# DeepRec-AI/DeepRec

Measured on AMD Instinct MI355X. Metric: samples/sec (whole node) DLRM Criteo-TB-shaped synthetic, higher is better.
Workload: dtype bf16; 1 GPU; model=dlrm, global_batch=8192, seq_len=1, parallelism=single, hip_graph=True, optimizer=adamasync, embedding_dim=16, num_tables=26

## Files before the change

deeprec_amd/ops/hip/dense_kernels.hip:

```cpp

#include <torch/extension.h>
#include <ATen/hip/HIPContext.h>
#include <hip/hip_runtime.h>
#include <hip/hip_bf16.h>

#include <algorithm>
#include <cstdint>

namespace py = pybind11;

static inline hipStream_t dense_stream() {
  return at::hip::getCurrentHIPStreamMasqueradingAsCUDA().stream();
}

namespace {

using bf16 = __hip_bfloat16;
using bf16x8 = __attribute__((ext_vector_type(8))) short;
using f32x4 = __attribute__((ext_vector_type(4))) float;

__device__ __forceinline__ float bf2f_u16(short u) {
  union {
    unsigned int i;
    float f;
  } cv;
  cv.i = ((unsigned int)(unsigned short)u) << 16;
  return cv.f;
}

__device__ __forceinline__ short f2bf_u16(float f) {
  union {
    float f;
    unsigned int i;
  } cv;
  cv.f = f;
  unsigned int lsb = (cv.i >> 16) & 1;
  cv.i += 0x7fff + lsb;
  return (short)(cv.i >> 16);
}

__device__ __forceinline__ short act_grad_u16(short g, short o, int act) {
  const float ov = bf2f_u16(o);
  if (act == 1) return ov > 0.0f ? g : (short)0;
  return f2bf_u16(bf2f_u16(g) * ov * (1.0f - ov));
}

__device__ __forceinline__ bf16x8 load_frag_row(const short* __restrict__ src,
                                                int r, int k0, int rows,
                                                int cols) {
  bf16x8 out;
  if (r < rows && k0 + 7 < cols) {
    const short* p = src + (int64_t)r * cols + k0;
    out = *reinterpret_cast<const bf16x8*>(p);
  } else {
#pragma unroll
    for (int i = 0; i < 8; ++i) {
      short v = 0;
      if (r < rows && k0 + i < cols) v = src[(int64_t)r * cols + k0 + i];
      out[i] = v;
    }
  }
  return out;
}

__device__ __forceinline__ bf16x8 load_frag_col(const short* __restrict__ src,
                                                int c, int k0, int rows,
                                                int cols) {
  bf16x8 out;
#pragma unroll
  for (int i = 0; i < 8; ++i) {
    short v = 0;
    int r = k0 + i;
    if (r < rows && c < cols) v = src[(int64_t)r * cols + c];
    out[i] = v;
  }
  return out;
}

template <int MT>
__global__ void k_linear_fwd_t(const short* __restrict__ A,
                               const short* __restrict__ W,
                               const float* __restrict__ bias, int M, int N,
                               int K, int act, short* __restrict__ C) {
  const int lane = threadIdx.x & 63;
  const int wave = threadIdx.x >> 6;
  const int ntiles64 = (N + 63) / 64;
  const int m0 = (blockIdx.x / ntiles64) * 64 * MT + wave * 16 * MT;
  const int n0 = (blockIdx.x % ntiles64) * 64;
  if (m0 >= M) return;
  const int col_b = n0 + (lane & 15);
  const int kgrp = (lane >> 4) * 8;
  f32x4 acc[MT][4] = {};
  const int nt = min(4, (N - n0 + 15) / 16);
  for (int k0 = 0; k0 < K; k0 += 32) {
    bf16x8 a[MT];
#pragma unroll
    for (int r = 0; r < MT; ++r)
      a[r] = load_frag_row(A, m0 + r * 16 + (lane & 15), k0 + kgrp, M, K);
#pragma unroll
    for (int t = 0; t < 4; ++t) {
      if (t >= nt) break;
      bf16x8 b = load_frag_row(W, col_b + t * 16, k0 + kgrp, N, K);
#pragma unroll
      for (int r = 0; r < MT; ++r)
        acc[r][t] = __builtin_amdgcn_mfma_f32_16x16x32_bf16(a[r], b,
                                                            acc[r][t], 0, 0,
                                                            0);
    }
  }
  __shared__ short cstage[4][16][72];
  const bool full_tile =
      (MT == 1) && (n0 + 64 <= N) && (m0 + 16 <= M) && ((N & 7) == 0);
  if (full_tile) {
#pragma unroll
    for (int t = 0; t < 4; ++t) {
      const int cn = t * 16 + (lane & 15);
      const float bv = bias ? bias[n0 + cn] : 0.0f;
#pragma unroll
      for (int i = 0; i < 4; ++i) {
        float v = acc[0][t][i] + bv;
        if (act == 1 && v < 0.0f) v = 0.0f;
        else if (act == 2) v = 1.0f / (1.0f + __expf(-v));
        cstage[wave][(lane >> 4) * 4 + i][cn] = f2bf_u16(v);
      }
    }
    __builtin_amdgcn_s_waitcnt(0);
#pragma unroll
    for (int half = 0; half < 2; ++half) {
      const int row = half * 8 + (lane >> 3);
      const int c8 = (lane & 7) * 8;
      bf16x8 vreg;
#pragma unroll
      for (int j = 0; j < 8; ++j) vreg[j] = cstage[wave][row][c8 + j];
      *reinterpret_cast<bf16x8*>(
          C + (int64_t)(m0 + row) * N + n0 + c8) = vreg;
    }
    return;
  }
#pragma unroll
  for (int r = 0; r < MT; ++r) {
#pragma unroll
    for (int t = 0; t < 4; ++t) {
      if (t >= nt) break;
      const int cn = n0 + t * 16 + (lane & 15);
      if (cn >= N) continue;
      const float bv = bias ? bias[cn] : 0.0f;
#pragma unroll
      for (int i = 0; i < 4; ++i) {
        int cm = m0 + r * 16 + (lane >> 4) * 4 + i;
        if (cm >= M) continue;
        float v = acc[r][t][i] + bv;
        if (act == 1 && v < 0.0f) v = 0.0f;
        else if (act == 2) v = 1.0f / (1.0f + __expf(-v));
        C[(int64_t)cm * N + cn] = f2bf_u16(v);
      }
    }
  }
}

__global__ void k_linear_dx(const short* __restrict__ G,
                            const short* __restrict__ W, int M, int N, int K,
                            short* __restrict__ dX,
                            const short* __restrict__ prev_out,
                            int prev_act) {
  const int lane = threadIdx.x & 63;
  const int wave = threadIdx.x >> 6;
  const int ktiles64 = (K + 63) / 64;
  const int m0 = (blockIdx.x / ktiles64) * 64 + wave * 16;
  const int c0 = (blockIdx.x % ktiles64) * 64;
  if (m0 >= M) return;
  const int row_g = m0 + (lane & 15);
  const int col_w = c0 + (lane & 15);
  const int kgrp = (lane >> 4) * 8;
  f32x4 acc[4] = {{0.f, 0.f, 0.f, 0.f}, {0.f, 0.f, 0.f, 0.f},
                  {0.f, 0.f, 0.f, 0.f}, {0.f, 0.f, 0.f, 0.f}};
  const int kt = min(4, (K - c0 + 15) / 16);
  for (int n0 = 0; n0 < N; n0 += 32) {
    bf16x8 a = load_frag_row(G, row_g, n0 + kgrp, M, N);
#pragma unroll
    for (int t = 0; t < 4; ++t) {
      if (t >= kt) break;
      bf16x8 b = load_frag_col(W, col_w + t * 16, n0 + kgrp, N, K);
      acc[t] = __builtin_amdgcn_mfma_f32_16x16x32_bf16(a, b, acc[t], 0, 0,
                                                       0);
    }
  }
#pragma unroll
  for (int t = 0; t < 4; ++t) {
    if (t >= kt) break;
    const int ck = c0 + t * 16 + (lane & 15);
    if (ck >= K) continue;
#pragma unroll
    for (int i = 0; i < 4; ++i) {
      int cm = m0 + (lane >> 4) * 4 + i;
      if (cm >= M) continue;
      short v = f2bf_u16(acc[t][i]);
      if (prev_out)
        v = act_grad_u16(v, prev_out[(int64_t)cm * K + ck], prev_act);
      dX[(int64_t)cm * K + ck] = v;
    }
  }
}

constexpr int DX_NSUP = 256;
__global__ void k_linear_dx_lds(const short* __restrict__ G,
                                const short* __restrict__ W, int M, int N,
                                int K, short* __restrict__ dX,
                                const short* __restrict__ prev_out,
                                int prev_act) {
  __shared__ short wl[64][DX_NSUP + 8];
  const int lane = threadIdx.x & 63;
  const int wave = threadIdx.x >> 6;
  const int ktiles64 = (K + 63) / 64;
  const int m0 = (blockIdx.x / ktiles64) * 128 + wave * 32;
  const int c0 = (blockIdx.x % ktiles64) * 64;
  const int row_g0 = m0 + (lane & 15);
  const int row_g1 = m0 + 16 + (lane & 15);
  const int kgrp = (lane >> 4) * 8;
  const int kt = min(4, (K - c0 + 15) / 16);
  f32x4 acc[2][4] = {};
  for (int ns = 0; ns < N; ns += DX_NSUP) {
    const int nlen = min(DX_NSUP, N - ns);
    __syncthreads();
    {
      const int r = threadIdx.x >> 3;
      const int seg = threadIdx.x & 7;
      const int nstg = (nlen + 31) & ~31;
      for (int it = 0; it * 32 < nstg; ++it) {
        int n = it * 32 + r;
        bf16x8 v = load_frag_row(W, ns + n, c0 + seg * 8, N, K);
#pragma unroll
        for (int j = 0; j < 8; ++j) wl[seg * 8 + j][n] = v[j];
      }
    }
    __syncthreads();
    if (m0 >= M) continue;
    for (int n0 = 0; n0 < nlen; n0 += 32) {
      bf16x8 a0 = load_frag_row(G, row_g0, ns + n0 + kgrp, M, N);
      bf16x8 a1 = load_frag_row(G, row_g1, ns + n0 + kgrp, M, N);
#pragma unroll
      for (int t = 0; t < 4; ++t) {
        if (t >= kt) break;
        bf16x8 b = *reinterpret_cast<const bf16x8*>(
            &wl[t * 16 + (lane & 15)][n0 + kgrp]);
        acc[0][t] =
            __builtin_amdgcn_mfma_f32_16x16x32_bf16(a0, b, acc[0][t], 0, 0,
                                                    0);
        acc[1][t] =
            __builtin_amdgcn_mfma_f32_16x16x32_bf16(a1, b, acc[1][t], 0, 0,
                                                    0);
      }
    }
  }
  if (m0 >= M) return;
#pragma unroll
  for (int rg = 0; rg < 2; ++rg) {
#pragma unroll
    for (int t = 0; t < 4; ++t) {
      if (t >= kt) break;
      const int ck = c0 + t * 16 + (lane & 15);
      if (ck >= K) continue;
#pragma unroll
      for (int i = 0; i < 4; ++i) {
        int cm = m0 + rg * 16 + (lane >> 4) * 4 + i;
        if (cm >= M) continue;
        short v = f2bf_u16(acc[rg][t][i]);
        if (prev_out)
          v = act_grad_u16(v, prev_out[(int64_t)cm * K + ck], prev_act);
        dX[(int64_t)cm * K + ck] = v;
      }
    }
  }
}

__global__ void k_linear_dw_lds(const short* __restrict__ G,
                                const short* __restrict__ A, int M, int N,
                                int K, float* __restrict__ dW,
                                float* __restrict__ dbias) {
  constexpr int CH = 128;
  constexpr int KG = 64;
  constexpr int APAD = 8;
  __shared__ short a_l[CH][KG + APAD];
  __shared__ short g_l[CH][16 + APAD];
  __shared__ float bred[16];

  const int lane = threadIdx.x & 63;
  const int wave = threadIdx.x >> 6;
  const int tid = threadIdx.x;
  const int kgroups = (K + KG - 1) / KG;
  const int tiles_n = (N + 15) / 16;
  const int tile_id = blockIdx.x % (tiles_n * kgroups);
  const int chunk = blockIdx.x / (tiles_n * kgroups);
  const int n0 = (tile_id / kgroups) * 16;
  const int k0 = (tile_id % kgroups) * KG;
  const int mbeg = chunk * CH;

  {
    const int r_in_iter = tid >> 3;
    const int seg = tid & 7;
    for (int it = 0; it < CH / 32; ++it) {
      int r = it * 32 + r_in_iter;
      int m = mbeg + r;
      bf16x8 v = load_frag_row(A, m, k0 + seg * 8, M, K);
      *reinterpret_cast<bf16x8*>(&a_l[r][seg * 8]) = v;
    }
    const int r_g = tid >> 1;
    const int seg_g = tid & 1;
    bf16x8 v = load_frag_row(G, mbeg + r_g, n0 + seg_g * 8, M, N);
    *reinterpret_cast<bf16x8*>(&g_l[r_g][seg_g * 8]) = v;
  }
  __syncthreads();

  const int kw = wave * 16;
  const int col_a = kw + (lane & 15);
  const int col_g = lane & 15;
  const int kgrp = (lane >> 4) * 8;
  f32x4 acc = {0.f, 0.f, 0.f, 0.f};
  float bsum = 0.0f;
  const bool do_bias = (dbias != nullptr) && (k0 == 0) && (wave == 0);
#pragma unroll
  for (int ms = 0; ms < CH; ms += 32) {
    bf16x8 afrag, gfrag;
#pragma unroll
    for (int i = 0; i < 8; ++i) {
      int m = ms + kgrp + i;
      gfrag[i] = g_l[m][col_g];
      afrag[i] = a_l[m][col_a];
    }
    acc = __builtin_amdgcn_mfma_f32_16x16x32_bf16(gfrag, afrag, acc, 0, 0,
                                                  0);
    if (do_bias) {
#pragma unroll
      for (int i = 0; i < 8; ++i) bsum += bf2f_u16(gfrag[i]);
    }
  }
  const int ck = k0 + col_a;
  if (ck < K) {
#pragma unroll
    for (int i = 0; i < 4; ++i) {
      int cn = n0 + (lane >> 4) * 4 + i;
      if (cn >= N) continue;
      atomicAdd(&dW[(int64_t)cn * K + ck], acc[i]);
    }
  }
  if (do_bias) {
    float v = bsum;
    for (int off = 16; off < 64; off += 16)
      v += __shfl(bsum, (lane & 15) + off);
    if (lane < 16) {
      int cn = n0 + lane;
      if (cn < N) atomicAdd(&dbias[cn], v);
    }
  }
}

__global__ void k_linear_dw_lds64(const short* __restrict__ G,
                                  const short* __restrict__ A, int M, int N,
                                  int K, float* __restrict__ dW,
                                  float* __restrict__ dbias) {
  constexpr int CH = 128;
  __shared__ short a_l[CH][64 + 8];
  __shared__ short g_l[CH][64 + 8];
  const int lane = threadIdx.x & 63;
  const int wave = threadIdx.x >> 6;
  const int tid = threadIdx.x;
  const int kgroups = (K + 63) / 64;
  const int ngroups = (N + 63) / 64;
  const int tile_id = blockIdx.x % (ngroups * kgroups);
  const int chunk = blockIdx.x / (ngroups * kgroups);
  const int n0 = (tile_id / kgroups) * 64;
  const int k0 = (tile_id % kgroups) * 64;
  const int mbeg = chunk * CH;
  {
    const int r = tid >> 3, seg = tid & 7;
    for (int it = 0; it < CH / 32; ++it) {
      int rr = it * 32 + r;
      *reinterpret_cast<bf16x8*>(&a_l[rr][seg * 8]) =
          load_frag_row(A, mbeg + rr, k0 + seg * 8, M, K);
      *reinterpret_cast<bf16x8*>(&g_l[rr][seg * 8]) =
          load_frag_row(G, mbeg + rr, n0 + seg * 8, M, N);
    }
  }
  __syncthreads();
  const int col_g = wave * 16 + (lane & 15);
  const int kgrp = (lane >> 4) * 8;
  f32x4 acc[4] = {};
  float bsum = 0.0f;
  const bool do_bias = (dbias != nullptr) && (k0 == 0);
#pragma unroll
  for (int ms = 0; ms < CH; ms += 32) {
    bf16x8 gfrag;
#pragma unroll
    for (int i = 0; i < 8; ++i) gfrag[i] = g_l[ms + kgrp + i][col_g];
    if (do_bias) {
#pragma unroll
      for (int i = 0; i < 8; ++i) bsum += bf2f_u16(gfrag[i]);
    }
#pragma unroll
    for (int t = 0; t < 4; ++t) {
      bf16x8 afrag;
#pragma unroll
      for (int i = 0; i < 8; ++i)
        afrag[i] = a_l[ms + kgrp + i][t * 16 + (lane & 15)];
      acc[t] =
          __builtin_amdgcn_mfma_f32_16x16x32_bf16(gfrag, afrag, acc[t], 0,
                                                  0, 0);
    }
  }
#pragma unroll
  for (int t = 0; t < 4; ++t) {
    const int ck = k0 + t * 16 + (lane & 15);
    if (ck >= K) continue;
#pragma unroll
    for (int i = 0; i < 4; ++i) {
      int cn = n0 + wave * 16 + (lane >> 4) * 4 + i;
      if (cn >= N) continue;
      atomicAdd(&dW[(int64_t)cn * K + ck], acc[t][i]);
    }
  }
  if (do_bias) {
    float v = bsum;
    for (int off = 16; off < 64; off += 16)
      v += __shfl(bsum, (lane & 15) + off);
    const int cn = n0 + wave * 16 + (lane & 15);
    if (lane < 16 && cn < N) atomicAdd(&dbias[cn], v);
  }
}

__global__ void k_linear_dw_lds64t(const short* __restrict__ G,
                                   const short* __restrict__ A, int M, int N,
                                   int K, int cpb,
                                   float* __restrict__ dW,
                                   float* __restrict__ dbias) {
  constexpr int CH = 128;
  __shared__ short a_t[64][CH + 8];
  __shared__ short g_t[64][CH + 8];
  const int lane = threadIdx.x & 63;
  const int wave = threadIdx.x >> 6;
  const int tid = threadIdx.x;
  const int kgroups = (K + 63) / 64;
  const int ngroups = (N + 63) / 64;
  const int tile_id = blockIdx.x % (ngroups * kgroups);
  const int chunk0 = (blockIdx.x / (ngroups * kgroups)) * cpb;
  const int n0 = (tile_id / kgroups) * 64;
  const int k0 = (tile_id % kgroups) * 64;
  const int col_g = wave * 16 + (lane & 15);
  const int kgrp = (lane >> 4) * 8;
  f32x4 acc[4] = {};
  float bsum = 0.0f;
  const bool do_bias = (dbias != nullptr) && (k0 == 0);
  for (int c = 0; c < cpb; ++c) {
    const int mbeg = (chunk0 + c) * CH;
    if (mbeg >= M) break;
    if (c > 0) __syncthreads();
    {
      const int r = tid >> 3, seg = tid & 7;
      for (int it = 0; it < CH / 32; ++it) {
        int rr = it * 32 + r;
        bf16x8 va = load_frag_row(A, mbeg + rr, k0 + seg * 8, M, K);
        bf16x8 vg = load_frag_row(G, mbeg + rr, n0 + seg * 8, M, N);
#pragma unroll
        for (int j = 0; j < 8; ++j) {
          a_t[seg * 8 + j][rr] = va[j];
          g_t[seg * 8 + j][rr] = vg[j];
        }
      }
    }
    __syncthreads();
#pragma unroll
    for (int ms = 0; ms < CH; ms += 32) {
      bf16x8 gfrag =
          *reinterpret_cast<const bf16x8*>(&g_t[col_g][ms + kgrp]);
      if (do_bias) {
#pragma unroll
        for (int i = 0; i < 8; ++i) bsum += bf2f_u16(gfrag[i]);
      }
#pragma unroll
      for (int t = 0; t < 4; ++t) {
        bf16x8 afrag = *reinterpret_cast<const bf16x8*>(
            &a_t[t * 16 + (lane & 15)][ms + kgrp]);
        acc[t] =
            __builtin_amdgcn_mfma_f32_16x16x32_bf16(gfrag, afrag, acc[t],
                                                    0, 0, 0);
      }
    }
  }
#pragma unroll
  for (int t = 0; t < 4; ++t) {
    const int ck = k0 + t * 16 + (lane & 15);
    if (ck >= K) continue;
#pragma unroll
    for (int i = 0; i < 4; ++i) {
      int cn = n0 + wave * 16 + (lane >> 4) * 4 + i;
      if (cn >= N) continue;
      atomicAdd(&dW[(int64_t)cn * K + ck], acc[t][i]);
    }
  }
  if (do_bias) {
    float v = bsum;
    for (int off = 16; off < 64; off += 16)
      v += __shfl(bsum, (lane & 15) + off);
    const int cn = n0 + wave * 16 + (lane & 15);
    if (lane < 16 && cn < N) atomicAdd(&dbias[cn], v);
  }
}

__device__ __forceinline__ float wave_sum(float v) {
#pragma unroll
  for (int off = 32; off; off >>= 1) v += __shfl_down(v, off);
  return __shfl(v, 0);
}

__global__ void k_l2norm_fwd(const short* __restrict__ X, int M, int N,
                             float eps, short* __restrict__ Y,
                             float* __restrict__ inv_norms) {
  const int lane = threadIdx.x & 63;
  const int row = blockIdx.x * 4 + (threadIdx.x >> 6);
  if (row >= M) return;
  const short* x = X + (int64_t)row * N;
  float ss = 0.0f;
  for (int j = lane; j < N; j += 64) {
    float v = bf2f_u16(x[j]);
    ss += v * v;
  }
  float inv = rsqrtf(fmaxf(wave_sum(ss), eps));
  short* y = Y + (int64_t)row * N;
  for (int j = lane; j < N; j += 64)
    y[j] = f2bf_u16(bf2f_u16(x[j]) * inv);
  if (lane == 0) inv_norms[row] = inv;
}

__global__ void k_l2norm_bwd(const short* __restrict__ dY,
                             const short* __restrict__ Y,
                             const float* __restrict__ inv_norms, int M,
                             int N, short* __restrict__ dX) {
  const int lane = threadIdx.x & 63;
  const int row = blockIdx.x * 4 + (threadIdx.x >> 6);
  if (row >= M) return;
  const short* dy = dY + (int64_t)row * N;
  const short* y = Y + (int64_t)row * N;
  float dot = 0.0f;
  for (int j = lane; j < N; j += 64)
    dot += bf2f_u16(y[j]) * bf2f_u16(dy[j]);
  dot = wave_sum(dot);
  const float inv = inv_norms[row];
  short* dx = dX + (int64_t)row * N;
  for (int j = lane; j < N; j += 64)
    dx[j] = f2bf_u16((bf2f_u16(dy[j]) - bf2f_u16(y[j]) * dot) * inv);
}

__global__ void k_zero_f32d(float* __restrict__ p, int64_t n) {
  const int64_t to16 =
      (int64_t)((16 - (reinterpret_cast<uintptr_t>(p) & 15)) & 15) >> 2;
  const int64_t head = to16 < n ? to16 : n;
  const int64_t nbody = (n - head) & ~3LL;
  float* body = p + head;
  int64_t i = (blockIdx.x * (int64_t)blockDim.x + threadIdx.x) * 4;
  int64_t stride = gridDim.x * (int64_t)blockDim.x * 4;
  for (; i < nbody; i += stride)
    *reinterpret_cast<float4*>(body + i) = make_float4(0.f, 0.f, 0.f, 0.f);
  if (blockIdx.x == 0 && threadIdx.x == 0) {
    for (int64_t j = 0; j < head; ++j) p[j] = 0.0f;
    for (int64_t j = head + nbody; j < n; ++j) p[j] = 0.0f;
  }
}

__global__ void k_dense_adam(float* __restrict__ w,
                             const float* __restrict__ g,
                             float* __restrict__ m, float* __restrict__ v,
                             short* __restrict__ w16,
                             const float* __restrict__ powers, int64_t n,
                             float lr, float beta1, float beta2, float eps,
                             float gscale) {
  const float lr_t = lr * sqrtf(1.0f - powers[1]) / (1.0f - powers[0]);
  int64_t i = blockIdx.x * (int64_t)blockDim.x + threadIdx.x;
  int64_t stride = gridDim.x * (int64_t)blockDim.x;
  for (; i < n; i += stride) {
    float gi = g[i] * gscale;
    float mn = beta1 * m[i] + (1.0f - beta1) * gi;
    float vn = beta2 * v[i] + (1.0f - beta2) * gi * gi;
    m[i] = mn;
    v[i] = vn;
    float wn = w[i] - lr_t * mn / (sqrtf(vn) + eps);
    w[i] = wn;
    if (w16) w16[i] = f2bf_u16(wn);
  }
}

template <int N>
__global__ void k_resln_fwd(const short* __restrict__ x,
                            const short* __restrict__ a,
                            const float* __restrict__ gamma,
                            const float* __restrict__ beta, int64_t M,
                            float eps, short* __restrict__ y,
                            short* __restrict__ z,
                            float* __restrict__ stats) {
  float gm[N], bt[N];
#pragma unroll
  for (int j = 0; j < N; ++j) {
    gm[j] = gamma[j];
    bt[j] = beta[j];
  }
  int64_t r = blockIdx.x * (int64_t)blockDim.x + threadIdx.x;
  int64_t stride = gridDim.x * (int64_t)blockDim.x;
  for (; r < M; r += stride) {
    const short* xp = x + r * N;
    const short* ap = a + r * N;
    float zv[N];
    float mean = 0.0f;
#pragma unroll
    for (int j = 0; j < N; ++j) {
      zv[j] = bf2f_u16(xp[j]) + bf2f_u16(ap[j]);
      mean += zv[j];
    }
    mean /= N;
    float var = 0.0f;
#pragma unroll
    for (int j = 0; j < N; ++j) {
      float d = zv[j] - mean;
      var += d * d;
    }
    float rstd = rsqrtf(var / N + eps);
    short* yp = y + r * N;
    short* zp = z + r * N;
#pragma unroll
    for (int j = 0; j < N; ++j) {
      zp[j] = f2bf_u16(zv[j]);
      yp[j] = f2bf_u16((zv[j] - mean) * rstd * gm[j] + bt[j]);
    }
    stats[r * 2] = mean;
    stats[r * 2 + 1] = rstd;
  }
}

template <int N>
__global__ void k_resln_bwd(const short* __restrict__ dy,
                            const short* __restrict__ z,
                            const float* __restrict__ stats,
                            const float* __restrict__ gamma, int64_t M,
                            short* __restrict__ dz,
                            float* __restrict__ dgamma,
                            float* __restrict__ dbeta) {
  __shared__ float ldg[N];
  __shared__ float ldb[N];
  for (int j = threadIdx.x; j < N; j += blockDim.x) {
    ldg[j] = 0.0f;
    ldb[j] = 0.0f;
  }
  __syncthreads();
  float gm[N], pg[N], pb[N];
#pragma unroll
  for (int j = 0; j < N; ++j) {
    gm[j] = gamma[j];
    pg[j] = 0.0f;
    pb[j] = 0.0f;
  }
  int64_t r = blockIdx.x * (int64_t)blockDim.x + threadIdx.x;
  int64_t stride = gridDim.x * (int64_t)blockDim.x;
  for (; r < M; r += stride) {
    const short* dyp = dy + r * N;
    const short* zp = z + r * N;
    const float mean = stats[r * 2];
    const float rstd = stats[r * 2 + 1];
    float s1 = 0.0f, s2 = 0.0f;
    float xh[N], g[N];
#pragma unroll
    for (int j = 0; j < N; ++j) {
      xh[j] = (bf2f_u16(zp[j]) - mean) * rstd;
      g[j] = bf2f_u16(dyp[j]);
      float gg = g[j] * gm[j];
      s1 += gg;
      s2 += gg * xh[j];
      pg[j] += g[j] * xh[j];
      pb[j] += g[j];
    }
    s1 /= N;
    s2 /= N;
    short* dzp = dz + r * N;
#pragma unroll
    for (int j = 0; j < N; ++j)
      dzp[j] = f2bf_u16((g[j] * gm[j] - s1 - xh[j] * s2) * rstd);
  }
#pragma unroll
  for (int j = 0; j < N; ++j) {
    atomicAdd(&ldg[j], pg[j]);
    atomicAdd(&ldb[j], pb[j]);
  }
  __syncthreads();
  for (int j = threadIdx.x; j < N; j += blockDim.x) {
    atomicAdd(&dgamma[j], ldg[j]);
    atomicAdd(&dbeta[j], ldb[j]);
  }
}

__global__ void k_act_bwd(const short* __restrict__ dY,
                          const short* __restrict__ out, int64_t n, int act,
                          short* __restrict__ G) {
  int64_t i = (blockIdx.x * (int64_t)blockDim.x + threadIdx.x) * 8;
  int64_t stride = gridDim.x * (int64_t)blockDim.x * 8;
  for (; i + 7 < n; i += stride) {
    bf16x8 g = *reinterpret_cast<const bf16x8*>(dY + i);
    bf16x8 o = *reinterpret_cast<const bf16x8*>(out + i);
    bf16x8 r;
#pragma unroll
    for (int j = 0; j < 8; ++j) r[j] = act_grad_u16(g[j], o[j], act);
    *reinterpret_cast<bf16x8*>(G + i) = r;
  }
  if (blockIdx.x == 0 && threadIdx.x == 0) {
    for (int64_t j = n & ~7LL; j < n; ++j)
      G[j] = act_grad_u16(dY[j], out[j], act);
  }
}

__global__ void k_pad_cast_bf16(const float* __restrict__ x, int64_t M, int K,
                                int KP, short* __restrict__ y) {
  const int gpr = (KP + 7) / 8;
  const int64_t ngroups = M * gpr;
  int64_t gi = blockIdx.x * (int64_t)blockDim.x + threadIdx.x;
  const int64_t stride = gridDim.x * (int64_t)blockDim.x;
  for (; gi < ngroups; gi += stride) {
    const int64_t r = gi / gpr;
    const int c0 = (int)(gi % gpr) * 8;
    bf16x8 v;
#pragma unroll
    for (int j = 0; j < 8; ++j) {
      short b = 0;
      if (c0 + j < K) {
        const float f = x[r * K + c0 + j];
        b = f != f ? (short)0x7fc0 : f2bf_u16(f);
      }
      v[j] = b;
    }
    short* dst = y + r * KP + c0;
    if ((KP & 7) == 0) {
      *reinterpret_cast<bf16x8*>(dst) = v;
    } else {
#pragma unroll
      for (int j = 0; j < 8; ++j)
        if (c0 + j < KP) dst[j] = v[j];
    }
  }
}

__global__ void k_interact_fwd(const short* __restrict__ feats, int B, int F,
                               int D, int P, int P_pad,
                               short* __restrict__ out) {
  const int lane = threadIdx.x & 63;
  const int wave = threadIdx.x >> 6;
  const int b = blockIdx.x * 4 + wave;
  extern __shared__ short lds[];
  short* f = lds + wave * F * D;
  const bool active = b < B;
  if (active) {
    const short* src = feats + (int64_t)b * F * D;
    for (int t = lane; t * 8 < F * D; t += 64) {
      *reinterpret_cast<bf16x8*>(f + t * 8) =
          *reinterpret_cast<const bf16x8*>(src + t * 8);
    }
  }
  __syncthreads();
  if (!active) return;
  short* dst = reinterpret_cast<short*>(out) + (int64_t)b * P_pad;
  for (int p = lane; p < P_pad; p += 64) {
    if (p >= P) {
      dst[p] = 0;
      continue;
    }
    int i = 0, rem = p, row = F - 1;
    while (rem >= row) {
      rem -= row;
      --row;
      ++i;
    }
    int j = i + 1 + rem;
    float acc = 0.0f;
    const short* fi = f + i * D;
    const short* fj = f + j * D;
    for (int d = 0; d < D; ++d)
      acc += bf2f_u16(fi[d]) * bf2f_u16(fj[d]);
    dst[p] = f2bf_u16(acc);
  }
}

__global__ void k_interact_cat_fwd(const short* __restrict__ bot,
                                   const short* __restrict__ emb, int B,
                                   int Fe, int D, int P, int P_pad,
                                   short* __restrict__ out) {
  const int lane = threadIdx.x & 63;
  const int wave = threadIdx.x >> 6;
  const int b = blockIdx.x * 4 + wave;
  const int F = Fe + 1;
  extern __shared__ short lds[];
  short* f = lds + wave * F * D;
  const bool active = b < B;
  if (active) {
    const short* bsrc = bot + (int64_t)b * D;
    for (int t = lane; t * 8 < D; t += 64)
      *reinterpret_cast<bf16x8*>(f + t * 8) =
          *reinterpret_cast<const bf16x8*>(bsrc + t * 8);
    const short* esrc = emb + (int64_t)b * Fe * D;
    for (int t = lane; t * 8 < Fe * D; t += 64)
      *reinterpret_cast<bf16x8*>(f + D + t * 8) =
          *reinterpret_cast<const bf16x8*>(esrc + t * 8);
  }
  __syncthreads();
  if (!active) return;
  short* dst = reinterpret_cast<short*>(out) + (int64_t)b * (D + P_pad);
  for (int d = lane; d < D; d += 64) dst[d] = f[d];
  dst += D;
  for (int p = lane; p < P_pad; p += 64) {
    if (p >= P) {
      dst[p] = 0;
      continue;
    }
    int i = 0, rem = p, row = F - 1;
    while (rem >= row) {
      rem -= row;
      --row;
      ++i;
    }
    int j = i + 1 + rem;
    float acc = 0.0f;
    const short* fi = f + i * D;
    const short* fj = f + j * D;
    for (int d = 0; d < D; ++d)
      acc += bf2f_u16(fi[d]) * bf2f_u16(fj[d]);
    dst[p] = f2bf_u16(acc);
  }
}

__global__ void k_interact_cat_bwd(const short* __restrict__ grad,
                                   const short* __restrict__ bot,
                                   const short* __restrict__ emb, int B,
                                   int Fe, int D, int P, int P_pad,
                                   short* __restrict__ dbot,
                                   short* __restrict__ demb) {
  const int lane = threadIdx.x & 63;
  const int wave = threadIdx.x >> 6;
  const int b = blockIdx.x * 4 + wave;
  const int F = Fe + 1;
  extern __shared__ short lds[];
  short* f = lds + wave * (F * D + ((P + 7) & ~7));
  short* g = f + F * D;
  const bool active = b < B;
  if (active) {
    const short* bsrc = bot + (int64_t)b * D;
    for (int t = lane; t * 8 < D; t += 64)
      *reinterpret_cast<bf16x8*>(f + t * 8) =
          *reinterpret_cast<const bf16x8*>(bsrc + t * 8);
    const short* esrc = emb + (int64_t)b * Fe * D;
    for (int t = lane; t * 8 < Fe * D; t += 64)
      *reinterpret_cast<bf16x8*>(f + D + t * 8) =
          *reinterpret_cast<const bf16x8*>(esrc + t * 8);
    const short* gsrc = grad + (int64_t)b * (D + P_pad) + D;
    for (int t = lane; t < P; t += 64) g[t] = gsrc[t];
  }
  __shared__ short plut[40 * 40];
  for (int t = threadIdx.x; t < F * F; t += blockDim.x) {
    int i = t / F, j = t % F;
    int lo = i < j ? i : j, hi = i < j ? j : i;
    plut[t] = (short)(i == j ? -1
                             : lo * F - (lo * (lo + 1)) / 2 + (hi - lo - 1));
  }
  __syncthreads();
  if (!active) return;
  const short* gdirect = grad + (int64_t)b * (D + P_pad);
  short* db = dbot + (int64_t)b * D;
  short* de = demb + (int64_t)b * Fe * D;
  for (int t = lane; t < F * D; t += 64) {
    int i = t / D, d = t % D;
    float acc = 0.0f;
    const short* prow = &plut[i * F];
    const short* fd = f + d;
#pragma unroll 4
    for (int j = 0; j < F; ++j) {
      int p = prow[j];
      if (p < 0) continue;
      acc += bf2f_u16(g[p]) * bf2f_u16(fd[j * D]);
    }
    if (i == 0) {
      db[d] = f2bf_u16(acc + bf2f_u16(gdirect[d]));
    } else {
      de[(i - 1) * D + d] = f2bf_u16(acc);
    }
  }
}

__global__ void k_interact_bwd(const short* __restrict__ grad,
                               const short* __restrict__ feats, int B, int F,
                               int D, int P, int P_pad,
                               short* __restrict__ dfeats) {
  const int lane = threadIdx.x & 63;
  const int wave = threadIdx.x >> 6;
  const int b = blockIdx.x * 4 + wave;
  extern __shared__ short lds[];
  short* f = lds + wave * (F * D + ((P + 7) & ~7));
  short* g = f + F * D;
  const bool active = b < B;
  if (active) {
    const short* fsrc = feats + (int64_t)b * F * D;
    const short* gsrc = grad + (int64_t)b * P_pad;
    for (int t = lane; t * 8 < F * D; t += 64)
      *reinterpret_cast<bf16x8*>(f + t * 8) =
          *reinterpret_cast<const bf16x8*>(fsrc + t * 8);
    for (int t = lane; t < P; t += 64) g[t] = gsrc[t];
  }
  __shared__ short plut[40 * 40];
  for (int t = threadIdx.x; t < F * F; t += blockDim.x) {
    int i = t / F, j = t % F;
    int lo = i < j ? i : j, hi = i < j ? j : i;
    plut[t] = (short)(i == j ? -1
                             : lo * F - (lo * (lo + 1)) / 2 + (hi - lo - 1));
  }
  __syncthreads();
  if (!active) return;
  short* dst = reinterpret_cast<short*>(dfeats) + (int64_t)b * F * D;
  for (int t = lane; t < F * D; t += 64) {
    int i = t / D, d = t % D;
    float acc = 0.0f;
    const short* prow = &plut[i * F];
    const short* fd = f + d;
#pragma unroll 4
    for (int j = 0; j < F; ++j) {
      int p = prow[j];
      if (p < 0) continue;
      acc += bf2f_u16(g[p]) * bf2f_u16(fd[j * D]);
    }
    dst[t] = f2bf_u16(acc);
  }
}

}


static const short* bf_ptr(const torch::Tensor& t) {
  return reinterpret_cast<const short*>(t.data_ptr<at::BFloat16>());
}
static short* bf_ptr_mut(torch::Tensor& t) {
  return reinterpret_cast<short*>(t.data_ptr<at::BFloat16>());
}

static void check_bf16_matrix(const torch::Tensor& t, const char* op,
                              const char* name) {
  TORCH_CHECK(t.is_cuda(), op, ": ", name, " must be on the GPU");
  TORCH_CHECK(t.dim() == 2, op, ": ", name, " must be 2-D, got ", t.dim(),
              "-D");
  TORCH_CHECK(t.scalar_type() == torch::kBFloat16, op, ": ", name,
              " must be bfloat16, got ", t.scalar_type());
  TORCH_CHECK(t.is_contiguous(), op, ": ", name,
              " must be contiguous (row-major)");
}

torch::Tensor linear_fwd(torch::Tensor x, torch::Tensor w_bf16,
                         torch::Tensor bias, int64_t act,
                         int64_t variant) {
  check_bf16_matrix(x, "linear_fwd", "x");
  check_bf16_matrix(w_bf16, "linear_fwd", "w");
  TORCH_CHECK(x.size(1) == w_bf16.size(1), "linear_fwd: x is [M,",
              x.size(1), "] but w is [N,", w_bf16.size(1), "]");
  int M = x.size(0), K = x.size(1), N = w_bf16.size(0);
  TORCH_CHECK(!bias.defined() || bias.numel() == 0 ||
                  (bias.numel() == N && bias.is_contiguous()),
              "linear_fwd: bias must be empty or contiguous [N]");
  auto out = torch::empty({M, N}, x.options());
  int tiles_n = (N + 63) / 64;
  const float* bp =
      bias.defined() && bias.numel() ? bias.data_ptr<float>() : nullptr;
  if (variant < 0) variant = 0;
  if (variant == 1) {
    int blocks = ((M + 127) / 128) * tiles_n;
    k_linear_fwd_t<2><<<blocks, 256, 0, dense_stream()>>>(
        bf_ptr(x), bf_ptr(w_bf16), bp, M, N, K, (int)act, bf_ptr_mut(out));
  } else {
    int blocks = ((M + 63) / 64) * tiles_n;
    k_linear_fwd_t<1><<<blocks, 256, 0, dense_stream()>>>(
        bf_ptr(x), bf_ptr(w_bf16), bp, M, N, K, (int)act, bf_ptr_mut(out));
  }
  return out;
}

torch::Tensor linear_dx(torch::Tensor g, torch::Tensor w_bf16,
                        c10::optional<torch::Tensor> prev_out,
                        int64_t prev_act) {
  check_bf16_matrix(g, "linear_dx", "g");
  check_bf16_matrix(w_bf16, "linear_dx", "w");
  TORCH_CHECK(g.size(1) == w_bf16.size(0), "linear_dx: g is [M,", g.size(1),
              "] but w is [", w_bf16.size(0), ",K]");
  int M = g.size(0), N = g.size(1), K = w_bf16.size(1);
  TORCH_CHECK(prev_act >= 0 && prev_act <= 2, "linear_dx: prev_act must be "
              "0 (none), 1 (relu) or 2 (sigmoid), got ", prev_act);
  const short* pp = nullptr;
  if (prev_out.has_value()) {
    check_bf16_matrix(*prev_out, "linear_dx", "prev_out");
    TORCH_CHECK(prev_out->size(0) == M && prev_out->size(1) == K,
                "linear_dx: prev_out is [", prev_out->size(0), ",",
                prev_out->size(1), "] but dX is [", M, ",", K, "]");
    if (prev_act != 0) pp = bf_ptr(*prev_out);
  } else {
    TORCH_CHECK(prev_act == 0, "linear_dx: prev_act without prev_out");
  }
  auto dx = torch::empty({M, K}, g.options());
  int tiles_k = (K + 63) / 64;
  if (N >= 128) {
    int blocks = ((M + 127) / 128) * tiles_k;
    k_linear_dx_lds<<<blocks, 256, 0, dense_stream()>>>(
        bf_ptr(g), bf_ptr(w_bf16), M, N, K, bf_ptr_mut(dx), pp,
        (int)prev_act);
  } else {
    int blocks = ((M + 63) / 64) * tiles_k;
    k_linear_dx<<<blocks, 256, 0, dense_stream()>>>(
        bf_ptr(g), bf_ptr(w_bf16), M, N, K, bf_ptr_mut(dx), pp,
        (int)prev_act);
  }
  return dx;
}

static void zero_f32_launch(float* p, int64_t n) {
  k_zero_f32d<<<(int)std::clamp<int64_t>((n / 4 + 255) / 256, 1, 1024), 256,
                0, dense_stream()>>>(p, n);
}

static std::tuple<torch::Tensor, torch::Tensor> linear_dw_impl(
    torch::Tensor g, torch::Tensor x, torch::Tensor ws, bool want_bias,
    int64_t variant, bool zero = true) {
  check_bf16_matrix(g, "linear_dw", "g");
  check_bf16_matrix(x, "linear_dw", "x");
  TORCH_CHECK(g.size(0) == x.size(0), "linear_dw: g has ", g.size(0),
              " rows but x has ", x.size(0));
  int M = g.size(0), N = g.size(1), K = x.size(1);
  int64_t ws_len = (int64_t)N * K + (want_bias ? N : 0);
  if (zero) zero_f32_launch(ws.data_ptr<float>(), ws_len);
  auto dw = ws.narrow(0, 0, (int64_t)N * K).view({N, K});
  auto db = want_bias ? ws.narrow(0, (int64_t)N * K, N) : torch::Tensor();
  int m_chunks = (M + 127) / 128;
  float* dbp = want_bias ? db.data_ptr<float>() : nullptr;
  if (variant < 0) variant = N >= 64 ? 2 : 0;
  if (variant == 2) {
    int tiles = ((N + 63) / 64) * ((K + 63) / 64);
    int cpb = std::max(1, (int)((int64_t)m_chunks * tiles / 512));
    int chunk_blocks = (m_chunks + cpb - 1) / cpb;
    k_linear_dw_lds64t<<<tiles * chunk_blocks, 256, 0, dense_stream()>>>(
        bf_ptr(g), bf_ptr(x), M, N, K, cpb, dw.data_ptr<float>(), dbp);
  } else if (variant == 1) {
    int tiles = ((N + 63) / 64) * ((K + 63) / 64);
    k_linear_dw_lds64<<<tiles * m_chunks, 256, 0, dense_stream()>>>(
        bf_ptr(g), bf_ptr(x), M, N, K, dw.data_ptr<float>(), dbp);
  } else {
    int tiles = ((N + 15) / 16) * ((K + 63) / 64);
    k_linear_dw_lds<<<tiles * m_chunks, 256, 0, dense_stream()>>>(
        bf_ptr(g), bf_ptr(x), M, N, K, dw.data_ptr<float>(), dbp);
  }
  return {dw, db};
}

std::tuple<torch::Tensor, torch::Tensor> linear_dw(torch::Tensor g,
                                                   torch::Tensor x,
                                                   bool want_bias,
                                                   int64_t variant) {
  check_bf16_matrix(g, "linear_dw", "g");
  check_bf16_matrix(x, "linear_dw", "x");
  int N = g.size(1), K = x.size(1);
  int64_t ws_len = (int64_t)N * K + (want_bias ? N : 0);
  auto ws = torch::empty({ws_len}, g.options().dtype(torch::kFloat32));
  return linear_dw_impl(g, x, ws, want_bias, variant);
}

std::tuple<torch::Tensor, torch::Tensor> linear_dw_out(torch::Tensor g,
                                                       torch::Tensor x,
                                                       torch::Tensor ws,
                                                       bool want_bias,
                                                       int64_t variant,
                                                       bool zero) {
  TORCH_CHECK(ws.is_cuda() && ws.is_contiguous() &&
              ws.scalar_type() == torch::kFloat32);
  check_bf16_matrix(g, "linear_dw_out", "g");
  check_bf16_matrix(x, "linear_dw_out", "x");
  int N = g.size(1), K = x.size(1);
  int64_t ws_len = (int64_t)N * K + (want_bias ? N : 0);
  TORCH_CHECK(ws.numel() == ws_len, "linear_dw_out: workspace size");
  return linear_dw_impl(g, x, ws, want_bias, variant, zero);
}

void zero_f32(torch::Tensor ws) {
  TORCH_CHECK(ws.is_cuda() && ws.dim() == 1 && ws.is_contiguous() &&
                  ws.scalar_type() == torch::kFloat32,
              "zero_f32: ws must be a contiguous 1-D fp32 GPU tensor");
  if (ws.numel() == 0) return;
  zero_f32_launch(ws.data_ptr<float>(), ws.numel());
}

torch::Tensor pad_cast_bf16(torch::Tensor x, int64_t k_pad) {
  TORCH_CHECK(x.is_cuda() && x.dim() == 2 && x.is_contiguous() &&
                  x.scalar_type() == torch::kFloat32,
              "pad_cast_bf16: x must be a contiguous 2-D fp32 GPU tensor");
  int64_t M = x.size(0), K = x.size(1);
  TORCH_CHECK(k_pad >= K, "pad_cast_bf16: k_pad ", k_pad, " < K ", K);
  TORCH_CHECK(k_pad < (1 << 30), "pad_cast_bf16: k_pad ", k_pad,
              " is out of range (< 2^30)");
  auto y = torch::empty({M, k_pad}, x.options().dtype(torch::kBFloat16));
  if (M == 0 || k_pad == 0) return y;
  int64_t groups = M * ((k_pad + 7) / 8);
  int blocks = (int)std::clamp<int64_t>((groups + 255) / 256, 1, 4096);
  k_pad_cast_bf16<<<blocks, 256, 0, dense_stream()>>>(
      x.data_ptr<float>(), M, (int)K, (int)k_pad, bf_ptr_mut(y));
  return y;
}

std::tuple<torch::Tensor, torch::Tensor, torch::Tensor> resln_fwd(
    torch::Tensor x, torch::Tensor a, torch::Tensor gamma,
    torch::Tensor beta, double eps) {
  TORCH_CHECK(x.scalar_type() == torch::kBFloat16 && x.is_contiguous());
  int64_t M = x.numel() / x.size(-1);
  int N = x.size(-1);
  TORCH_CHECK(N <= 64, "resln: row width must be <= 64");
  auto y = torch::empty_like(x);
  auto z = torch::empty_like(x);
  auto stats = torch::empty({M, 2}, x.options().dtype(torch::kFloat32));
  if (M == 0) return {y, z, stats};
  TORCH_CHECK(N == 16 || N == 32 || N == 64, "resln: N must be 16/32/64");
  int blocks = (int)std::min<int64_t>((M + 255) / 256, 4096);
#define RESLN_FWD(NV) \
  k_resln_fwd<NV><<<blocks, 256, 0, dense_stream()>>>( \
      bf_ptr(x), bf_ptr(a), gamma.data_ptr<float>(), \
      beta.data_ptr<float>(), M, (float)eps, bf_ptr_mut(y), \
      bf_ptr_mut(z), stats.data_ptr<float>())
  if (N == 16) RESLN_FWD(16);
  else if (N == 32) RESLN_FWD(32);
  else RESLN_FWD(64);
#undef RESLN_FWD
  return {y, z, stats};
}

std::tuple<torch::Tensor, torch::Tensor, torch::Tensor> resln_bwd(
    torch::Tensor dy, torch::Tensor z, torch::Tensor stats,
    torch::Tensor gamma) {
  int64_t M = z.numel() / z.size(-1);
  int N = z.size(-1);
  auto dz = torch::empty_like(z);
  auto opts = gamma.options();
  auto dgamma = torch::empty({N}, opts);
  auto dbeta = torch::empty({N}, opts);
  auto stream = dense_stream();
  k_zero_f32d<<<1, 64, 0, stream>>>(dgamma.data_ptr<float>(), N);
  k_zero_f32d<<<1, 64, 0, stream>>>(dbeta.data_ptr<float>(), N);
  if (M == 0) return {dz, dgamma, dbeta};
  auto dyc = dy.contiguous();
  int blocks = (int)std::min<int64_t>((M + 256 * 8 - 1) / (256 * 8), 4096);
  blocks = std::max(blocks, 64);
#define RESLN_BWD(NV) \
  k_resln_bwd<NV><<<blocks, 256, 0, stream>>>( \
      bf_ptr(dyc), bf_ptr(z), stats.data_ptr<float>(), \
      gamma.data_ptr<float>(), M, bf_ptr_mut(dz), \
      dgamma.data_ptr<float>(), dbeta.data_ptr<float>())
  if (N == 16) RESLN_BWD(16);
  else if (N == 32) RESLN_BWD(32);
  else RESLN_BWD(64);
#undef RESLN_BWD
  return {dz, dgamma, dbeta};
}

void dense_adam(torch::Tensor w, torch::Tensor g, torch::Tensor m,
                torch::Tensor v, torch::Tensor w16, torch::Tensor powers,
                double lr, double beta1, double beta2, double eps,
                double gscale) {
  int64_t n = w.numel();
  if (n == 0) return;
  short* w16p = (w16.defined() && w16.numel())
                    ? reinterpret_cast<short*>(w16.data_ptr<at::BFloat16>())
                    : nullptr;
  int blocks = (int)std::min<int64_t>((n + 255) / 256, 4096);
  k_dense_adam<<<blocks, 256, 0, dense_stream()>>>(
      w.data_ptr<float>(), g.data_ptr<float>(), m.data_ptr<float>(),
      v.data_ptr<float>(), w16p, powers.data_ptr<float>(), n, (float)lr,
      (float)beta1, (float)beta2, (float)eps, (float)gscale);
}

torch::Tensor act_bwd(torch::Tensor dy, torch::Tensor out, int64_t act) {
  auto g = torch::empty_like(dy);
  int64_t n = dy.numel();
  int blocks = (int)std::min<int64_t>((n / 8 + 255) / 256, 4096);
  k_act_bwd<<<std::max(blocks, 1), 256, 0, dense_stream()>>>(
      bf_ptr(dy), bf_ptr(out), n, (int)act, bf_ptr_mut(g));
  return g;
}

torch::Tensor interact_fwd(torch::Tensor feats, int64_t p_pad) {
  TORCH_CHECK(feats.scalar_type() == torch::kBFloat16 &&
              feats.is_contiguous());
  int B = feats.size(0), F = feats.size(1), D = feats.size(2);
  int P = F * (F - 1) / 2;
  TORCH_CHECK((F * D) % 8 == 0, "F*D must be a multiple of 8");
  auto out = torch::empty({B, p_pad}, feats.options());
  int blocks = (B + 3) / 4;
  size_t lds = 4 * (size_t)F * D * sizeof(short);
  k_interact_fwd<<<blocks, 256, lds, dense_stream()>>>(
      bf_ptr(feats), B, F, D, P, (int)p_pad, bf_ptr_mut(out));
  return out;
}

torch::Tensor interact_bwd(torch::Tensor grad, torch::Tensor feats) {
  int B = feats.size(0), F = feats.size(1), D = feats.size(2);
  TORCH_CHECK(F <= 40, "interact_bwd: pair LUT supports F <= 40");
  int P = F * (F - 1) / 2;
  int P_pad = grad.size(1);
  auto dfeats = torch::empty_like(feats);
  int blocks = (B + 3) / 4;
  size_t lds = 4 * (size_t)(F * D + ((P + 7) & ~7)) * sizeof(short);
  k_interact_bwd<<<blocks, 256, lds, dense_stream()>>>(
      bf_ptr(grad.contiguous()), bf_ptr(feats), B, F, D, P, P_pad,
      bf_ptr_mut(dfeats));
  return dfeats;
}

torch::Tensor interact_cat_fwd(torch::Tensor bot, torch::Tensor emb,
                               int64_t p_pad) {
  TORCH_CHECK(bot.scalar_type() == torch::kBFloat16 && bot.is_contiguous());
  TORCH_CHECK(emb.scalar_type() == torch::kBFloat16 && emb.is_contiguous());
  int B = emb.size(0), Fe = emb.size(1), D = emb.size(2);
  int F = Fe + 1;
  int P = F * (F - 1) / 2;
  TORCH_CHECK(D % 8 == 0, "D must be a multiple of 8");
  auto out = torch::empty({B, D + p_pad}, emb.options());
  int blocks = (B + 3) / 4;
  size_t lds = 4 * (size_t)F * D * sizeof(short);
  k_interact_cat_fwd<<<blocks, 256, lds, dense_stream()>>>(
      bf_ptr(bot), bf_ptr(emb), B, Fe, D, P, (int)p_pad, bf_ptr_mut(out));
  return out;
}

std::tuple<torch::Tensor, torch::Tensor> interact_cat_bwd(
    torch::Tensor grad, torch::Tensor bot, torch::Tensor emb) {
  int B = emb.size(0), Fe = emb.size(1), D = emb.size(2);
  int F = Fe + 1;
  TORCH_CHECK(F <= 40, "interact: pair LUT supports F <= 40");
  int P = F * (F - 1) / 2;
  int P_pad = grad.size(1) - D;
  auto dbot = torch::empty_like(bot);
  auto demb = torch::empty_like(emb);
  int blocks = (B + 3) / 4;
  size_t lds = 4 * (size_t)(F * D + ((P + 7) & ~7)) * sizeof(short);
  k_interact_cat_bwd<<<blocks, 256, lds, dense_stream()>>>(
      bf_ptr(grad.contiguous()), bf_ptr(bot), bf_ptr(emb), B, Fe, D, P,
      P_pad, bf_ptr_mut(dbot), bf_ptr_mut(demb));
  return {dbot, demb};
}

std::tuple<torch::Tensor, torch::Tensor> l2norm_fwd(torch::Tensor x,
                                                    double eps) {
  TORCH_CHECK(x.scalar_type() == torch::kBFloat16 && x.is_contiguous());
  int M = x.size(0), N = x.size(1);
  auto y = torch::empty_like(x);
  auto inv = torch::empty({M}, x.options().dtype(torch::kFloat32));
  k_l2norm_fwd<<<(M + 3) / 4, 256, 0, dense_stream()>>>(
      bf_ptr(x), M, N, (float)eps, bf_ptr_mut(y), inv.data_ptr<float>());
  return {y, inv};
}

torch::Tensor l2norm_bwd(torch::Tensor dy, torch::Tensor y,
                         torch::Tensor inv) {
  int M = y.size(0), N = y.size(1);
  auto dx = torch::empty_like(y);
  k_l2norm_bwd<<<(M + 3) / 4, 256, 0, dense_stream()>>>(
      bf_ptr(dy.contiguous()), bf_ptr(y), inv.data_ptr<float>(), M, N,
      bf_ptr_mut(dx));
  return dx;
}

void register_dense(py::module_& mod) {
  mod.def("l2norm_fwd", &l2norm_fwd);
  mod.def("l2norm_bwd", &l2norm_bwd);
  mod.def("interact_fwd", &interact_fwd);
  mod.def("interact_bwd", &interact_bwd);
  mod.def("interact_cat_fwd", &interact_cat_fwd);
  mod.def("interact_cat_bwd", &interact_cat_bwd);
  mod.def("linear_fwd", &linear_fwd, py::arg("x"), py::arg("w"),
          py::arg("bias"), py::arg("act"), py::arg("variant") = -1);
  mod.def("linear_dx", &linear_dx, py::arg("g"), py::arg("w"),
          py::arg("prev_out") = py::none(), py::arg("prev_act") = 0);
  mod.def("linear_dw", &linear_dw, py::arg("g"), py::arg("x"),
          py::arg("want_bias"), py::arg("variant") = -1);
  mod.def("linear_dw_out", &linear_dw_out, py::arg("g"), py::arg("x"),
          py::arg("ws"), py::arg("want_bias"), py::arg("variant") = -1,
          py::arg("zero") = true);
  mod.def("zero_f32", &zero_f32, py::arg("ws"));
  mod.def("pad_cast_bf16", &pad_cast_bf16, py::arg("x"), py::arg("k_pad"));
  mod.def("dense_adam", &dense_adam);
  mod.def("resln_fwd", &resln_fwd);
  mod.def("resln_bwd", &resln_bwd);
  mod.def("act_bwd", &act_bwd);
}
```

Measured before the change: 13.86 million samples/sec.

## Use transposing LDS reads with swizzled row-major staging in dX and dW kernels

```diff
diff --git a/deeprec_amd/ops/hip/dense_kernels.hip b/deeprec_amd/ops/hip/dense_kernels.hip
--- a/deeprec_amd/ops/hip/dense_kernels.hip
+++ b/deeprec_amd/ops/hip/dense_kernels.hip
@@ -75,6 +75,29 @@
     out[i] = v;
   }
   return out;
+}
+
+using bf16x4 = __attribute__((ext_vector_type(4))) short;
+constexpr int TRT_COLS = 64;
+
+__device__ __forceinline__ int trt_off(int row, int col) {
+  const int sw = ((row >> 1) & 1) | ((row >> 2) & 2);
+  return row * TRT_COLS + ((((col >> 4) ^ sw) << 4) | (col & 15));
+}
+
+__device__ __forceinline__ int trt_lane_off(int lane, int cb) {
+  return trt_off(8 * (lane >> 4) + ((lane >> 2) & 3), cb + 4 * (lane & 3));
+}
+
+__device__ __forceinline__ bf16x4 lds_read_tr16(const short* p) {
+  return __builtin_amdgcn_ds_read_tr16_b64_v4i16(
+      (__attribute__((address_space(3))) bf16x4*)p);
+}
+
+__device__ __forceinline__ bf16x8 trt_frag(const short* p) {
+  const bf16x4 lo = lds_read_tr16(p);
+  const bf16x4 hi = lds_read_tr16(p + 4 * TRT_COLS);
+  return __builtin_shufflevector(lo, hi, 0, 1, 2, 3, 4, 5, 6, 7);
 }
 
 template <int MT>
@@ -203,14 +226,15 @@
 }
 
 constexpr int DX_NSUP = 256;
+constexpr int DX_STAGE_BATCH = 2;
 __global__ void k_linear_dx_lds(const short* __restrict__ G,
                                 const short* __restrict__ W, int M, int N,
                                 int K, short* __restrict__ dX,
                                 const short* __restrict__ prev_out,
                                 int prev_act) {
-  __shared__ short wl[64][DX_NSUP + 8];
+  __shared__ __attribute__((aligned(16))) short wl[DX_NSUP * TRT_COLS];
   const int lane = threadIdx.x & 63;
-  const int wave = threadIdx.x >> 6;
+  const int wave = __builtin_amdgcn_readfirstlane(threadIdx.x >> 6);
   const int ktiles64 = (K + 63) / 64;
   const int m0 = (blockIdx.x / ktiles64) * 128 + wave * 32;
   const int c0 = (blockIdx.x % ktiles64) * 64;
@@ -218,19 +242,28 @@
   const int row_g1 = m0 + 16 + (lane & 15);
   const int kgrp = (lane >> 4) * 8;
   const int kt = min(4, (K - c0 + 15) / 16);
+  const int st_r = threadIdx.x >> 3;
+  const int st_seg = threadIdx.x & 7;
+  const int st_off = trt_off(st_r, st_seg * 8);
+  int b_off[4];
+#pragma unroll
+  for (int t = 0; t < 4; ++t) b_off[t] = trt_lane_off(lane, t * 16);
   f32x4 acc[2][4] = {};
   for (int ns = 0; ns < N; ns += DX_NSUP) {
     const int nlen = min(DX_NSUP, N - ns);
     __syncthreads();
     {
-      const int r = threadIdx.x >> 3;
-      const int seg = threadIdx.x & 7;
       const int nstg = (nlen + 31) & ~31;
-      for (int it = 0; it * 32 < nstg; ++it) {
-        int n = it * 32 + r;
-        bf16x8 v = load_frag_row(W, ns + n, c0 + seg * 8, N, K);
-#pragma unroll
-        for (int j = 0; j < 8; ++j) wl[seg * 8 + j][n] = v[j];
+      for (int it0 = 0; it0 * 32 < nstg; it0 += DX_STAGE_BATCH) {
+        bf16x8 v[DX_STAGE_BATCH];
+#pragma unroll
+        for (int j = 0; j < DX_STAGE_BATCH; ++j)
+          v[j] = load_frag_row(W, ns + (it0 + j) * 32 + st_r,
+                               c0 + st_seg * 8, N, K);
+#pragma unroll
+        for (int j = 0; j < DX_STAGE_BATCH; ++j)
+          *reinterpret_cast<bf16x8*>(
+              &wl[(it0 + j) * 32 * TRT_COLS + st_off]) = v[j];
       }
     }
     __syncthreads();
@@ -241,8 +274,7 @@
 #pragma unroll
       for (int t = 0; t < 4; ++t) {
         if (t >= kt) break;
-        bf16x8 b = *reinterpret_cast<const bf16x8*>(
-            &wl[t * 16 + (lane & 15)][n0 + kgrp]);
+        bf16x8 b = trt_frag(&wl[n0 * TRT_COLS + b_off[t]]);
         acc[0][t] =
             __builtin_amdgcn_mfma_f32_16x16x32_bf16(a0, b, acc[0][t], 0, 0,
                                                     0);
@@ -433,8 +465,8 @@
                                    float* __restrict__ dW,
                                    float* __restrict__ dbias) {
   constexpr int CH = 128;
-  __shared__ short a_t[64][CH + 8];
-  __shared__ short g_t[64][CH + 8];
+  __shared__ __attribute__((aligned(16))) short a_s[CH * TRT_COLS];
+  __shared__ __attribute__((aligned(16))) short g_s[CH * TRT_COLS];
   const int lane = threadIdx.x & 63;
   const int wave = threadIdx.x >> 6;
   const int tid = threadIdx.x;
@@ -444,8 +476,12 @@
   const int chunk0 = (blockIdx.x / (ngroups * kgroups)) * cpb;
   const int n0 = (tile_id / kgroups) * 64;
   const int k0 = (tile_id % kgroups) * 64;
-  const int col_g = wave * 16 + (lane & 15);
-  const int kgrp = (lane >> 4) * 8;
+  const int st_r = tid >> 3, st_seg = tid & 7;
+  const int st_off = trt_off(st_r, st_seg * 8);
+  const int g_off = trt_lane_off(lane, wave * 16);
+  int a_off[4];
+#pragma unroll
+  for (int t = 0; t < 4; ++t) a_off[t] = trt_lane_off(lane, t * 16);
   f32x4 acc[4] = {};
   float bsum = 0.0f;
   const bool do_bias = (dbias != nullptr) && (k0 == 0);
@@ -453,32 +489,29 @@
     const int mbeg = (chunk0 + c) * CH;
     if (mbeg >= M) break;
     if (c > 0) __syncthreads();
-    {
-      const int r = tid >> 3, seg = tid & 7;
-      for (int it = 0; it < CH / 32; ++it) {
-        int rr = it * 32 + r;
-        bf16x8 va = load_frag_row(A, mbeg + rr, k0 + seg * 8, M, K);
-        bf16x8 vg = load_frag_row(G, mbeg + rr, n0 + seg * 8, M, N);
-#pragma unroll
-        for (int j = 0; j < 8; ++j) {
-          a_t[seg * 8 + j][rr] = va[j];
-          g_t[seg * 8 + j][rr] = vg[j];
-        }
-      }
+    bf16x8 va[CH / 32], vg[CH / 32];
+#pragma unroll
+    for (int it = 0; it < CH / 32; ++it) {
+      const int m = mbeg + it * 32 + st_r;
+      va[it] = load_frag_row(A, m, k0 + st_seg * 8, M, K);
+      vg[it] = load_frag_row(G, m, n0 + st_seg * 8, M, N);
+    }
+#pragma unroll
+    for (int it = 0; it < CH / 32; ++it) {
+      *reinterpret_cast<bf16x8*>(&a_s[it * 32 * TRT_COLS + st_off]) = va[it];
+      *reinterpret_cast<bf16x8*>(&g_s[it * 32 * TRT_COLS + st_off]) = vg[it];
     }
     __syncthreads();
 #pragma unroll
     for (int ms = 0; ms < CH; ms += 32) {
-      bf16x8 gfrag =
-          *reinterpret_cast<const bf16x8*>(&g_t[col_g][ms + kgrp]);
+      bf16x8 gfrag = trt_frag(&g_s[ms * TRT_COLS + g_off]);
       if (do_bias) {
 #pragma unroll
         for (int i = 0; i < 8; ++i) bsum += bf2f_u16(gfrag[i]);
       }
 #pragma unroll
       for (int t = 0; t < 4; ++t) {
-        bf16x8 afrag = *reinterpret_cast<const bf16x8*>(
-            &a_t[t * 16 + (lane & 15)][ms + kgrp]);
+        bf16x8 afrag = trt_frag(&a_s[ms * TRT_COLS + a_off[t]]);
         acc[t] =
             __builtin_amdgcn_mfma_f32_16x16x32_bf16(gfrag, afrag, acc[t],
                                                     0, 0, 0);
```

Result: faster. 14.96 million samples/sec, median of 6 (+7.9%).
